# z430/keyword-spotting

Measured on AMD Instinct MI355X. Metric: 1s 16kHz clips/sec end-to-end (wav->label), higher is better.
Workload: dtype f32

## Files before the change

keyword-spotting_amd/csrc/kws_api.hip:

```cpp
#include <atomic>
#include <chrono>
#include <cmath>
#include <cstdio>
#include <cstring>
#include <new>

#include "kws_ctx.h"

namespace kws {

const char* const kKernelNames[KWS_K_COUNT] = {"kws_mfcc_i16_kernel", "kws_dscnn_fwd_kernel", "kws_cnntrad_conv_kernel",
                                               "kws_cnntrad_dense_kernel", "kws_stream_frame_kernel", "kws_mfcc_f64_kernel",
                                               "kws_mfcc_refine_kernel"};


static double hz2mel(double hz) { return 2595.0 * std::log10(1.0 + hz / 700.0); }
static double mel2hz(double mel) { return 700.0 * (std::pow(10.0, mel / 2595.0) - 1.0); }

static void mel_edges(int nfilt, int nfft, int sample_rate, std::vector<int>& edges) {
    const double lowmel = hz2mel(0.0), highmel = hz2mel(sample_rate / 2.0);
    const int num = nfilt + 2;
    const double step = (highmel - lowmel) / (double)(num - 1);
    edges.resize(num);
    for (int i = 0; i < num; ++i) {
// ... 151 lines not shown
    KWS_GUARD_BEGIN
    if (!out) return fail(nullptr, KWS_EINVAL, "kws_create: out is NULL");
    *out = nullptr;
    int ndev = 0;
    hipError_t e = hipGetDeviceCount(&ndev);
    if (e != hipSuccess || ndev <= 0)
        return fail(nullptr, KWS_EHIP, std::string("kws_create: no HIP device (") + hipGetErrorString(e) + "); there is no CPU fallback");
    if (device_id < 0 || device_id >= ndev) return fail(nullptr, KWS_EINVAL, "kws_create: device_id out of range");
    kws_ctx* c = new (std::nothrow) kws_ctx();
    if (!c) return fail(nullptr, KWS_ENOMEM, "kws_create: out of host memory");
    c->device = device_id;
    e = hipSetDevice(device_id);
    if (e == hipSuccess) e = hipStreamCreateWithFlags(&c->own_stream, hipStreamNonBlocking);
    if (e == hipSuccess) e = dscnn_init_device();
    if (e == hipSuccess) e = cnntrad_init_device();
    if (e != hipSuccess) {
        int rc = fail_hip(nullptr, e, "kws_create");
        if (c->own_stream) (void)hipStreamDestroy(c->own_stream);
        delete c;
        return rc;
    }
    c->stream = c->own_stream;
    int rc = kws_set_frontend(c, 16000, 16000, 400, 160, 512, 26, 10, 0.97f, 22);
    if (rc != KWS_OK) {
        g_create_err = c->err;
        kws_destroy(c);
        return rc;
    }
    *out = c;
    return KWS_OK;
// ... 543 lines not shown
    if (rc) return rc;
    if (!d_logits) return fail(c, KWS_EINVAL, std::string(fn) + ": d_logits is NULL");
    if (!c->model_ready) return fail(c, KWS_ESTATE, std::string(fn) + ": no model loaded (kws_load_dscnn)");
    HIP_TRY(c, hipSetDevice(c->device));
    if (c->mw.in_channels > 1) {
        if (d_act || d_stamps || (mode != KWS_PW_SPLIT_BF16 && mode != KWS_PW_PAIR_F16))
            return fail(c, KWS_EUNSUPPORTED, std::string(fn) + ": input_channels > 1 runs on the product kernels only");
        rc = grow_conv_ws(c, (size_t)B * 64 * 141, fn);
        if (rc) return rc;
        HIP_TRY(c, launch_conv1_general(c->stream, d_feat, B, c->mw.in_channels, c->mw.c1_general, c->mw.c1_b, c->d_conv_ws));
        ProfScope ps(c, KWS_K_DSCNN);
        HIP_TRY(c, launch_dscnn(c->stream, c->mw, c->d_conv_ws, B, d_logits, d_label, nullptr, mode, nullptr, nullptr, true));
        return KWS_OK;
    }
    ProfScope ps(c, KWS_K_DSCNN);
    HIP_TRY(c, launch_dscnn(c->stream, c->mw, d_feat, B, d_logits, d_label, d_act, mode, d_stamps));
    return KWS_OK;
}

int kws_forward_f32(kws_ctx* c, const float* d_feat, int B, float* d_logits, int32_t* d_label) {
    return forward_impl(c, d_feat, B, d_logits, d_label, nullptr, c ? c->pw_math : 0, "kws_forward_f32");
}

static int forward_map_impl(kws_ctx* c, const float* d_feat, int B, int T, int F, float* d_logits, int32_t* d_label, float* d_layers,
                            const char* fn) {
    int rc = check_batch(c, d_feat, B, fn);
    if (rc) return rc;
    if (!d_logits) return fail(c, KWS_EINVAL, std::string(fn) + ": d_logits is NULL");
    if (!c->model_ready) return fail(c, KWS_ESTATE, std::string(fn) + ": no model loaded (kws_load_dscnn)");
    if (T == IN_T && F == IN_F && !d_layers) return forward_impl(c, d_feat, B, d_logits, d_label, nullptr, c->pw_math, fn);
    if (T < 6 || F < 6) return fail(c, KWS_EINVAL, std::string(fn) + ": the 10 x 10 first convolution (padding 2) needs T >= 6 and F >= 6");
// ... 1030 lines not shown
```

keyword-spotting_amd/csrc/kws_ctx.h:

```cpp
#pragma once
#include <new>

#include "kws_internal.h"

namespace kws {
struct Ingest;
void ingest_free(kws_ctx* c);
}

using kws::FrontendParams; using kws::FrontendTables; using kws::DscnnWeights; using kws::CnnTradWeights; using kws::NFFT;

struct kws_ctx {
    int device = 0;
    hipStream_t own_stream = nullptr;
    hipStream_t stream = nullptr;
    hipEvent_t order_ev = nullptr;
    std::string err;

    int sample_rate = 16000, nfft = NFFT, ceplifter = 22;
    FrontendParams fp{};
    bool fe_ready = false;
    bool fe_fast_ok = false;
    int fe_math = KWS_FE_F32;
    void* d_fe = nullptr;
    FrontendTables ft{};
    double* d_spec_tw64 = nullptr;
    int spec_nfft = 0;
    float refine_span = KWS_FE_REFINE_SPAN_DEFAULT;
// ... 88 lines not shown
```

keyword-spotting_amd/csrc/kws_dscnn.hip:

```cpp
#include <type_traits>

#include "kws_internal.h"
#include "kws_mfcc_dev.h"
#include "kws_split_mfma.h"

namespace kws {
namespace {


#ifndef KWS_DSCNN_WAVES
#define KWS_DSCNN_WAVES 8
#endif
#ifndef KWS_X_DSCNN_STAMP_TID
#define KWS_X_DSCNN_STAMP_TID 0
#endif
constexpr int NW = KWS_DSCNN_WAVES;
constexpr int NT = NW * 64;
constexpr int TW = 30;

constexpr int P0 = C1_H * C1_W;
constexpr int FEAT_H = 103, FEAT_W = 14;
constexpr int OFF_Z3 = 0, OFF_Z2 = 22976, OFF_Z1 = 0, OFF_Z0 = 9152, OFF_FEAT = 18304;
constexpr int OFF_DWTAB = 38784;
constexpr int OFF_PWB = OFF_DWTAB + 2 * 768;
// ... 23 lines not shown

#ifndef KWS_DSCNN_KSPLIT_LEFTOVER
#define KWS_DSCNN_KSPLIT_LEFTOVER 1
#endif
template <int N>
struct Leftover {
    static constexpr bool HAS = KWS_DSCNN_KSPLIT_LEFTOVER && (N == 1 || N == 2);
    static constexpr int TILE = N == 1 ? 4 : 8;
    static constexpr int P0T = TILE * TW;
    static constexpr int NP = HAS ? Blk<N>::POUT - P0T : 1;
    static constexpr int WAVE0 = N == 1 ? 4 : 0;
    static constexpr int OFF_PART = N == 1 ? OFF_Z2 : OFF_Z0;
};
static_assert(Blk<1>::TILES == 5 && Blk<2>::TILES == 9, "the leftover tiles are the fifth of block 1 and the ninth of block 2");
static_assert(4 * CH * Leftover<1>::NP <= 38784 - OFF_Z2 && OFF_Z0 + 4 * CH * Leftover<2>::NP <= OFF_FEAT, "partial sums fit their dead planes");

template <bool TO_MFMA = false>
__device__ __forceinline__ float stencil3x3(float w0, float w1, float w2, float w3, float w4, float w5, float w6,
                                            float w7, float w8, float b, float up, float mid, float dn, float mask_l,
                                            float mask_r) {
    float c, to_right, to_left;
    asm("v_mul_f32 %1, %3, %13\n\t"
        "v_mul_f32 %2, %5, %13\n\t"
        "v_fma_f32 %0, %4, %13, %12\n\t"
        "v_fmac_f32 %1, %6, %14\n\t"
        "v_fmac_f32 %2, %8, %14\n\t"
        "v_fmac_f32 %0, %7, %14\n\t"
        "v_fmac_f32 %1, %9, %15\n\t"
        "v_fmac_f32 %2, %11, %15\n\t"
        "v_fmac_f32 %0, %10, %15\n\t"
// ... 281 lines not shown
                const int oo = (ct ^ 1) * 32 + row_of(r, half);
                const float u0 = relu(fmaf(w.c1_b[oo], sig0, occ[r])), u1 = relu(fmaf(w.c1_b[oo + 1], sig0, occ[r + 1]));
                *reinterpret_cast<float2*>(z0 + pidx(oo, pos, P0 + 2)) = make_float2(u0, u1);
                if constexpr (PAIR) mx = fmaxf(mx, fmaxf(u0, u1));
            }
        }
    }
}

constexpr int C1W_ROWS = FEAT_H;
constexpr int OFF_C1W8 = OFF_Z1;
constexpr int OFF_C1P2 = OFF_C1W8 + 2 * C1W_ROWS * 3 * 4;
static_assert(OFF_C1P2 + 2 * C1W_ROWS * 3 <= OFF_Z0, "conv1's operand windows live where block 1's output goes later");
static_assert(2 * (C1_W - 1) + 9 < FEAT_W && 2 * (C1_H - 1) + 9 < FEAT_H, "window reach inside the padded map");

__device__ __forceinline__ void conv1_build_windows(float* lds, int tid, float sx) {
    const float* featp = lds + OFF_FEAT;
    uint32_t* w8 = reinterpret_cast<uint32_t*>(lds + OFF_C1W8);
    uint32_t* p2 = reinterpret_cast<uint32_t*>(lds + OFF_C1P2);
    for (int i = tid; i < C1W_ROWS * 3; i += NT) {
        const float* src = featp + (i / 3) * FEAT_W + 2 * (i % 3);
        const float y[8] = {src[0], src[1], src[2], src[3], src[4], src[5], src[6], src[7]};
        uintx4 hi, lo;
        split_pair8(y, sx, hi, lo);
        *reinterpret_cast<uintx4*>(w8 + i * 4) = hi;
        *reinterpret_cast<uintx4*>(w8 + (C1W_ROWS * 3 + i) * 4) = lo;
        uint32_t h, l;
        split_pair2(src[8], src[9], sx, h, l);
        p2[i] = h;
        p2[C1W_ROWS * 3 + i] = l;
    }
}
// ... 71 lines not shown
                const float c0 = (r & 2) ? o4.z : o4.x, c1 = (r & 2) ? o4.w : o4.y;
                const float u0 = relu(fmaf(c0, sig0, occ[r])), u1 = relu(fmaf(c1, sig0, occ[r + 1]));
                *reinterpret_cast<float2*>(z0 + pidx(oo, pos, P0 + 2)) = make_float2(u0, u1);
                mx = fmaxf(mx, fmaxf(u0, u1));
            }
        }
    }
}

struct PosRange {
    int lo, hi;
};

template <bool RANGED, int NP>
__device__ __forceinline__ void conv1_phase_split(const DscnnWeights& w, float* lds, int tid, const uintx4 (&c1f)[7][NP],
                                                  PosRange rg, float sx = 1.f, float sig0 = 1.f) {
    static_assert(P0 > 4 * 32 && P0 <= 5 * 32 && NW >= 6, "conv1 work split: four dual tiles + one tile in two halves");
    const float* featp = lds + OFF_FEAT;
    float* z0 = lds + OFF_Z0;
    const int lane = tid & 63, wv = tid >> 6;
    float mx = 0.f;
    if constexpr (NP == 2) {
        if constexpr (RANGED) {
            const int n_pt = (rg.hi - rg.lo + 31) / 32;
            for (int u = wv; u < 2 * n_pt; u += NW) conv1_unit_pairwin<false>(w, lds, z0, u >> 1, u & 1, lane, c1f, rg.lo, rg.hi, sig0, mx);
        } else if (wv < 4)
            conv1_unit_pairwin<true>(w, lds, z0, wv, wv & 1, lane, c1f, 0, P0, sig0, mx);
        else if (wv < 6)
            conv1_unit_pairwin<false>(w, lds, z0, 4, wv & 1, lane, c1f, 0, P0, sig0, mx);
    } else if constexpr (RANGED) {
        const int n_pt = (rg.hi - rg.lo + 31) / 32;
        for (int u = wv; u < 2 * n_pt; u += NW) conv1_unit_split<false, NP>(w, featp, z0, u >> 1, u & 1, lane, c1f, rg.lo, rg.hi, sx, sig0, mx);
    } else if (wv < 4)
// ... 82 lines not shown
    const float* pwb = lds + OFF_PWB + G::BUF * 64;
    float* zout = lds + G::OFF_OUT;
    float mx = 0.f;
    for (int i = tid; i < CH * L::NP; i += NT) {
        const int co = i / L::NP, j = i - co * L::NP;
        const float s = (part[i] + part[CH * L::NP + i]) + (part[2 * CH * L::NP + i] + part[3 * CH * L::NP + i]);
        const float v = relu(s + pwb[co]);
        zout[pidx(co, L::P0T + j, G::SOUT)] = v;
        mx = fmaxf(mx, v);
    }
    if constexpr (PAIR) publish_wave_max(lds, N == 1 ? 3 : 1, tid >> 6, tid & 63, mx);
}

template <int N, int MODE, bool RANGED = false>
__device__ __forceinline__ void block_phase(const DscnnWeights& w, float* lds, int tid, PwOperands<MODE>& pwo,
                                            float* __restrict__ act4 = nullptr, PosRange rg = PosRange{0, 0}, PairCtx pc = PairCtx{}) {
    using G = Blk<N>;
    constexpr bool PAIR = MODE == 5;
    constexpr int NP = PAIR ? 2 : 3;
    constexpr int NPROD = PAIR ? 3 : 6;
    constexpr bool KSL = Leftover<N>::HAS && (MODE == 4 || MODE == 5) && !RANGED;
    const int p_lo = RANGED ? rg.lo : 0, p_hi = RANGED ? rg.hi : G::POUT;
#ifdef KWS_X_DSCNN_SKIP_LEFTOVER
    const int n_tiles = RANGED ? (p_hi - p_lo + TW - 1) / TW : (N == 2 ? 8 : G::TILES);
#else
    const int n_tiles = RANGED ? (p_hi - p_lo + TW - 1) / TW : (KSL ? Leftover<N>::TILE : G::TILES);
#endif
    constexpr bool MFMA = MODE != 0;
    constexpr bool SPLIT = MODE >= 4;
    constexpr bool NO_STENCIL = MODE == 6;
    const int lane = tid & 63, wv = tid >> 6, half = lane >> 5, col = lane & 31;
    float* zout = lds + G::OFF_OUT;
    const float* dwtab = lds + OFF_DWTAB + G::BUF * 768;
    const float* pwb = lds + OFF_PWB + G::BUF * 64;
    float* poolbuf = lds + OFF_POOLBUF;

    BlockTables next_tables;
    if constexpr (N < 4) {
        fetch_block_tables(w, N + 1, tid, next_tables);
        if (tid < CH) {
            zout[pidx(tid, G::POUT, G::SOUT)] = relu(pwb[tid]);
            zout[pidx(tid, G::POUT + 1, G::SOUT)] = 0.f;
        }
    } else if (!MFMA) {
        poolbuf[wv * CH + lane] = 0.f;
    }

    const float4* bias4 = reinterpret_cast<const float4*>(pwb) + half;
    const float4* dwt4 = reinterpret_cast<const float4*>(dwtab) + half * 24;
    float psum[2][16];
// ... 340 lines not shown
                    "v_add_f32_dpp %12, %12, %12 row_bcast:15 row_mask:0xa bank_mask:0xf\n\t"
                    "v_add_f32_dpp %13, %13, %13 row_bcast:15 row_mask:0xa bank_mask:0xf\n\t"
                    "v_add_f32_dpp %14, %14, %14 row_bcast:15 row_mask:0xa bank_mask:0xf\n\t"
                    "v_add_f32_dpp %15, %15, %15 row_bcast:15 row_mask:0xa bank_mask:0xf"
                    : "+v"(q[0]), "+v"(q[1]), "+v"(q[2]), "+v"(q[3]), "+v"(q[4]), "+v"(q[5]), "+v"(q[6]), "+v"(q[7]), "+v"(q[8]), "+v"(q[9]), "+v"(q[10]), "+v"(q[11]), "+v"(q[12]), "+v"(q[13]), "+v"(q[14]), "+v"(q[15]));
            }
            if (col == 31) {
#pragma unroll
                for (int k = 0; k < 32; ++k) poolbuf[wv * CH + (k >> 4) * 32 + row_of(k & 15, half)] = psum[k >> 4][k & 15] * pc.inv_out;
            }
        }
    }
    (void)bias4;
}


template <int MODE, bool DIAG = true, bool PRECONV = false, bool STREAM = false, bool CLUSTER = false>
__global__ __launch_bounds__(NT) void kws_dscnn_fwd_kernel(DscnnWeights w, const float* __restrict__ feat, int B,
                                                           float* __restrict__ logits, int32_t* __restrict__ label,
                                                           float* __restrict__ act_arg,
                                                           unsigned long long* __restrict__ stamps_arg,
                                                           const int* __restrict__ ring_hops, StreamPush sp) {
    static_assert(!STREAM || (MODE >= 4 && !DIAG && !PRECONV), "the fused push exists for the product paths only");
    constexpr bool PAIR = MODE == 5;
    constexpr int NP = PAIR ? 2 : 3;
    BlockTables t1_pre{};
    static_assert(!CLUSTER || STREAM, "time-tile clusters exist for the streaming push only");
    float* const act = DIAG ? act_arg : nullptr;
    unsigned long long* const stamps = DIAG ? stamps_arg : nullptr;
    extern __shared__ __attribute__((aligned(16))) float lds[];
    constexpr bool MFMA = MODE != 0;
    const int tid = threadIdx.x;
    const int lane = tid & 63, wv = tid >> 6;

    const int cl_n = CLUSTER ? sp.cluster : 1;
    const int clip = CLUSTER ? (int)blockIdx.x / cl_n : (int)blockIdx.x;
    const int cl_tile = CLUSTER ? (int)blockIdx.x - clip * cl_n : 0;
    if (clip >= B) return;
    const int j0 = Blk<4>::H * cl_tile / cl_n, j1 = Blk<4>::H * (cl_tile + 1) / cl_n;
    auto rows = [&](int lo, int hi, int H, int W) { return PosRange{(lo < 0 ? 0 : lo) * W, (hi > H ? H : hi) * W}; };
    const PosRange rg4 = rows(j0, j1, Blk<4>::H, Blk<4>::W), rg3 = rows(j0 - 2, j1, Blk<3>::H, Blk<3>::W),
                   rg2 = rows(j0 - 4, j1, Blk<2>::H, Blk<2>::W), rg1 = rows(j0 - 6, j1, Blk<1>::H, Blk<1>::W),
                   rg0 = rows(j0 - 7, j1 + 1, C1_H, C1_W);
    int n_stamp = 0;
    auto stamp = [&]() {
        if (stamps && tid == KWS_X_DSCNN_STAMP_TID) stamps[(size_t)clip * KWS_DSCNN_STAMPS + n_stamp] = __builtin_amdgcn_s_memtime();
        ++n_stamp;
    };
    if (stamps && tid == KWS_X_DSCNN_STAMP_TID) stamps[(size_t)clip * KWS_DSCNN_STAMPS + KWS_DSCNN_STAMPS - 2] = __builtin_amdgcn_s_memrealtime();
    stamp();

    constexpr bool SPLIT = MODE >= 4;
    PwOperands<MODE> wa;
    int hops_before = 0;
    int kx = 0, ky[5] = {0, 0, 0, 0, 0}, sg[5] = {0, 0, 0, 0, 0};
    if constexpr (PRECONV) {
        static_assert(!PRECONV || MODE >= 4, "the pre-convolved entry exists for the product (split) path only");
        const float* z = feat + (size_t)clip * (CH * P0);
        fetch_block_tables(w, 1, tid, t1_pre);
        float zmax = 0.f;
        for (int i = tid; i < CH * P0; i += NT) {
            const float v = z[i];
            lds[OFF_Z0 + pidx(i / P0, i % P0, P0 + 2)] = v;
            zmax = fmaxf(zmax, v);
        }
        if (tid < CH) {
            lds[OFF_Z0 + pidx(tid, P0, P0 + 2)] = 0.f;
            lds[OFF_Z0 + pidx(tid, P0 + 1, P0 + 2)] = 0.f;
        }
        if constexpr (PAIR)
            publish_wave_max(lds, 1, wv, lane, zmax);
// ... 20 lines not shown
        if (f_start >= 0) row_new = (int)((((f_start / step) - head) % IN_T + IN_T) % IN_T);
    } else {
        head = ring_hops ? (((*ring_hops + 1 - sp.frames_lag) % IN_T) + IN_T) % IN_T : 0;
    }
#pragma unroll
    for (int k = 0; k < FV; ++k) {
        const int i = tid + k * NT;
        fv[k] = (i < IN_T * IN_F && i / IN_F != row_new) ? f[((i / IN_F + head) % IN_T) * IN_F + i % IN_F] : 0.f;
    }
    BlockTables t1;
    fetch_block_tables(w, 1, tid, t1);
    __builtin_amdgcn_sched_barrier(0);
    float a1[SPLIT ? 1 : 50];
    uintx4 c1f[SPLIT ? 7 : 1][NP];
    if constexpr (SPLIT) {
        const uintx4* src = reinterpret_cast<const uintx4*>(PAIR ? w.c1_pair : w.c1_split) + (size_t)(wv & 1) * (7 * NP * 64) + lane;
#pragma unroll
        for (int kb = 0; kb < 7; ++kb)
#pragma unroll
            for (int p = 0; p < NP; ++p) c1f[kb][p] = src[(kb * NP + p) * 64];
    } else if constexpr (MFMA) {
        const int half = lane >> 5, col = lane & 31, ct = wv & 1;
#pragma unroll
        for (int s = 0; s < 50; ++s) a1[s] = w.c1_w[(2 * s + half) * CH + ct * 32 + col];
        load_pointwise(w, 1, lane, wa);
    }
    __builtin_amdgcn_sched_barrier(0);
    if constexpr (PAIR) {
        float m = 0.f;
#pragma unroll
        for (int k = 0; k < FV; ++k) m = fmaxf(m, fabsf(fv[k]));
        publish_wave_max(lds, 0, wv, lane, m);
    }
    if constexpr (STREAM) {
#ifdef KWS_X_STREAM_NO_FRAME
// ... 134 lines not shown
        pc.s_pwb = pow2f(sg[4]);
    }
    block_phase<3, MODE, CLUSTER>(w, lds, tid, wa, nullptr, rg3, pc);
    stamp();
    __syncthreads();
    stamp();
    if (a) {
        const float u = PAIR ? pow2f(-sg[3]) : 1.f;
        for (int i = tid; i < CH * Blk<3>::POUT; i += NT)
            a[i] = lds[OFF_Z3 + pidx(i / Blk<3>::POUT, i % Blk<3>::POUT, Blk<3>::SOUT)] * u;
        a += CH * Blk<3>::POUT;
    }
    if constexpr (PAIR) {
        pc.inv_out = pow2f(-sg[4]);
    }
    block_phase<4, MODE, CLUSTER>(w, lds, tid, wa, a ? a + CH : nullptr, rg4, pc);
    stamp();
    const int C = w.num_classes;
    float4 fcw[CH / 4];
    float fcb = 0.f, ring_b = 0.f;
    if (wv == 0 && lane < C) {
        const float4* wr = reinterpret_cast<const float4*>(w.fc_w + lane * CH);
#pragma unroll
        for (int c = 0; c < CH / 4; ++c) fcw[c] = wr[c];
        fcb = w.fc_b[lane];
    }
    if (tid < CH) ring_b = w.pw_b[3 * CH + tid];
    __syncthreads();
    stamp();

    float* pooled = lds + OFF_POOLED;
    constexpr float RING_N = 55.f * 11.f - 53.f * 9.f;
// ... 44 lines not shown
            const float4* pl = reinterpret_cast<const float4*>(pooled);
#pragma unroll
            for (int c = 0; c < CH / 4; ++c) {
                const float4 a4 = fcw[c], p4 = pl[c];
                acc = fmaf(a4.x, p4.x, acc);
                acc = fmaf(a4.y, p4.y, acc);
                acc = fmaf(a4.z, p4.z, acc);
                acc = fmaf(a4.w, p4.w, acc);
            }
            logits[(size_t)clip * C + lane] = acc;
            if constexpr (STREAM) {
                if (sp.h_logits) __hip_atomic_store(sp.h_logits + (size_t)clip * C + lane, acc, __ATOMIC_RELAXED, __HIP_MEMORY_SCOPE_SYSTEM);
            }
            v = acc;
        }
        float m = v;
        m = fmaxf(m, __builtin_bit_cast(float, __builtin_amdgcn_update_dpp(__builtin_bit_cast(int, m), __builtin_bit_cast(int, m), 0x111, 0xf, 0xf, false)));
        m = fmaxf(m, __builtin_bit_cast(float, __builtin_amdgcn_update_dpp(__builtin_bit_cast(int, m), __builtin_bit_cast(int, m), 0x112, 0xf, 0xf, false)));
        m = fmaxf(m, __builtin_bit_cast(float, __builtin_amdgcn_update_dpp(__builtin_bit_cast(int, m), __builtin_bit_cast(int, m), 0x114, 0xf, 0xf, false)));
        m = fmaxf(m, __builtin_bit_cast(float, __builtin_amdgcn_update_dpp(__builtin_bit_cast(int, m), __builtin_bit_cast(int, m), 0x118, 0xf, 0xf, false)));
        m = fmaxf(m, __builtin_bit_cast(float, __builtin_amdgcn_update_dpp(__builtin_bit_cast(int, m), __builtin_bit_cast(int, m), 0x142, 0xa, 0xf, false)));
        m = fmaxf(m, __builtin_bit_cast(float, __builtin_amdgcn_update_dpp(__builtin_bit_cast(int, m), __builtin_bit_cast(int, m), 0x143, 0xc, 0xf, false)));
        const float vmax = __builtin_bit_cast(float, __builtin_amdgcn_readlane(__builtin_bit_cast(int, m), 63));
        const unsigned long long holders = __ballot(lane < C && v == vmax);
        const int idx = holders ? __ffsll(holders) - 1 : 0;
        if (label && lane == 0) label[clip] = idx;
        if constexpr (STREAM) {
            if (sp.h_label && lane == 0) __hip_atomic_store(sp.h_label + clip, idx, __ATOMIC_RELAXED, __HIP_MEMORY_SCOPE_SYSTEM);
        }
    }
    if constexpr (STREAM) {
        int finishers = (int)gridDim.x;
        if constexpr (CLUSTER) finishers /= cl_n;
        if (sp.h_flag) asm volatile("s_waitcnt vmcnt(0)" ::: "memory");
        if (run_fc && tid == 0 && atomicAdd(&sp.hops[1], 1) == finishers - 1) {
            sp.hops[1] = 0;
            sp.hops[0] = hops_before + 1;
            if (sp.h_flag) __hip_atomic_store(sp.h_flag, hops_before + 1, __ATOMIC_RELAXED, __HIP_MEMORY_SCOPE_SYSTEM);
        }
    }
    stamp();
    if (stamps && tid == KWS_X_DSCNN_STAMP_TID) stamps[(size_t)clip * KWS_DSCNN_STAMPS + KWS_DSCNN_STAMPS - 1] = __builtin_amdgcn_s_memrealtime();
}

}

hipError_t dscnn_init_device() {
    const int lds = LDS_FLOATS * (int)sizeof(float);
    const void* kernels[] = {reinterpret_cast<const void*>(kws_dscnn_fwd_kernel<0>), reinterpret_cast<const void*>(kws_dscnn_fwd_kernel<1>),
                             reinterpret_cast<const void*>(kws_dscnn_fwd_kernel<2>), reinterpret_cast<const void*>(kws_dscnn_fwd_kernel<3>),
                             reinterpret_cast<const void*>(kws_dscnn_fwd_kernel<4>), reinterpret_cast<const void*>(kws_dscnn_fwd_kernel<6>),
                             reinterpret_cast<const void*>(kws_dscnn_fwd_kernel<4, false>),
                             reinterpret_cast<const void*>(kws_dscnn_fwd_kernel<4, false, true>),
                             reinterpret_cast<const void*>(kws_dscnn_fwd_kernel<4, false, false, true>),
                             reinterpret_cast<const void*>(kws_dscnn_fwd_kernel<4, false, false, true, true>),
                             reinterpret_cast<const void*>(kws_dscnn_fwd_kernel<5>), reinterpret_cast<const void*>(kws_dscnn_fwd_kernel<5, false>),
                             reinterpret_cast<const void*>(kws_dscnn_fwd_kernel<5, false, true>),
                             reinterpret_cast<const void*>(kws_dscnn_fwd_kernel<5, false, false, true>),
                             reinterpret_cast<const void*>(kws_dscnn_fwd_kernel<5, false, false, true, true>)};
    for (const void* k : kernels) {
        hipError_t e = hipFuncSetAttribute(k, hipFuncAttributeMaxDynamicSharedMemorySize, lds);
        if (e != hipSuccess) return e;
    }
    return hipSuccess;
}

namespace {
__global__ __launch_bounds__(NT) void kws_conv1_general_kernel(const float* __restrict__ x, int C_in, const float* __restrict__ wt,
                                                               const float* __restrict__ bias, float* __restrict__ out) {
    __shared__ float plane[FEAT_H * FEAT_W];
    const int tid = threadIdx.x, co = tid & 63, g = tid >> 6;
    constexpr int PER = (P0 + NW - 1) / NW;
    float acc[PER];
#pragma unroll
// ... 44 lines not shown
            hipLaunchKernelGGL((kws_dscnn_fwd_kernel<4, false, false, true, true>), dim3(n_streams * sp.cluster), dim3(NT), lds, s, w, d_feat_ring,
                               n_streams, d_logits, d_label, nullptr, nullptr, nullptr, sp);
    } else {
        if (pair)
            hipLaunchKernelGGL((kws_dscnn_fwd_kernel<5, false, false, true>), dim3(n_streams), dim3(NT), lds, s, w, d_feat_ring, n_streams, d_logits,
                               d_label, nullptr, nullptr, nullptr, sp);
        else
            hipLaunchKernelGGL((kws_dscnn_fwd_kernel<4, false, false, true>), dim3(n_streams), dim3(NT), lds, s, w, d_feat_ring, n_streams, d_logits,
                               d_label, nullptr, nullptr, nullptr, sp);
    }
    return hipGetLastError();
}

hipError_t launch_dscnn(hipStream_t s, const DscnnWeights& w, const float* d_feat, int B, float* d_logits,
                        int32_t* d_label, float* d_act, int mode, unsigned long long* d_stamps, const int* d_ring_hops,
                        bool preconv, int frames_lag) {
    const size_t lds = LDS_FLOATS * sizeof(float);
    StreamPush lag{};
    lag.frames_lag = frames_lag;
    const int grid = B;
    if (preconv) {
        if (mode == 5)
            hipLaunchKernelGGL((kws_dscnn_fwd_kernel<5, false, true>), dim3(grid), dim3(NT), lds, s, w, d_feat, B, d_logits, d_label, nullptr, nullptr, nullptr, StreamPush{});
        else
            hipLaunchKernelGGL((kws_dscnn_fwd_kernel<4, false, true>), dim3(grid), dim3(NT), lds, s, w, d_feat, B, d_logits, d_label, nullptr, nullptr, nullptr, StreamPush{});
        return hipGetLastError();
    }
    switch (mode) {
        case 0: hipLaunchKernelGGL(kws_dscnn_fwd_kernel<0>, dim3(grid), dim3(NT), lds, s, w, d_feat, B, d_logits, d_label, d_act, d_stamps, d_ring_hops, lag); break;
        case 2: hipLaunchKernelGGL(kws_dscnn_fwd_kernel<2>, dim3(grid), dim3(NT), lds, s, w, d_feat, B, d_logits, d_label, d_act, d_stamps, d_ring_hops, lag); break;
        case 3: hipLaunchKernelGGL(kws_dscnn_fwd_kernel<3>, dim3(grid), dim3(NT), lds, s, w, d_feat, B, d_logits, d_label, d_act, d_stamps, d_ring_hops, lag); break;
        case 4:
            if (d_act || d_stamps)
                hipLaunchKernelGGL((kws_dscnn_fwd_kernel<4, true>), dim3(grid), dim3(NT), lds, s, w, d_feat, B, d_logits, d_label, d_act, d_stamps, d_ring_hops, lag);
            else
// ... 141 lines not shown
```

keyword-spotting_amd/csrc/kws_internal.h:

```cpp
#pragma once
#include <hip/hip_runtime.h>
#include <stdint.h>

#include <string>
#include <vector>

#include "kws_hip.h"

namespace kws {

constexpr int NFFT = 512;
constexpr int NBINS = NFFT / 2 + 1;
constexpr int MEL_CHUNK = 8;
constexpr int MEL_STRIDE = 10;
#ifndef KWS_MFCC_WAVES
#define KWS_MFCC_WAVES 4
#endif
#ifndef KWS_MFCC_PAIRS_PER_WAVE
#define KWS_MFCC_PAIRS_PER_WAVE 3
#endif
constexpr int MFCC_WAVES = KWS_MFCC_WAVES;
constexpr int MFCC_THREADS = MFCC_WAVES * 64;
constexpr int MFCC_FRAMES_PER_WG = 2 * KWS_MFCC_PAIRS_PER_WAVE * MFCC_WAVES;
constexpr int MAX_NFILT = 64;
// ... 115 lines not shown
    int ring_len;
    int* hops;
    int* refine_ctr;
    int frames_lag;
    int cluster;
    float* cl_part;
    int* cl_count;
    float* h_logits;
    int32_t* h_label;
    int* h_flag;
};
hipError_t launch_dscnn_stream(hipStream_t s, const DscnnWeights& w, const StreamPush& sp, float* d_feat_ring, int n_streams,
                               float* d_logits, int32_t* d_label, bool pair);
hipError_t launch_dscnn(hipStream_t s, const DscnnWeights& w, const float* d_feat, int B, float* d_logits,
                        int32_t* d_label, float* d_act, int mode, unsigned long long* d_stamps = nullptr,
                        const int* d_ring_hops = nullptr, bool preconv = false, int frames_lag = 3);
hipError_t launch_conv1_general(hipStream_t s, const float* d_x, int B, int C_in, const float* d_wt, const float* d_bias, float* d_out);

struct CnnTradWeights {
    const uint32_t* c1_split;
    const float* c1_b;
    const uint32_t* c2_split;
    const float* c2_b;
    const uint32_t* lin_split;
    const float* lin_b;
    const float* dnn_w;
    const float* dnn_b;
    const float* fc_w;
    const float* fc_b;
    int num_classes;
    const uint32_t* c1_h2;
// ... 31 lines not shown
```

Measured before the change: 6.941 million.

## Run DS-CNN forward as persistent workgroups that prefetch the next clip

```diff
diff --git a/keyword-spotting_amd/csrc/kws_api.hip b/keyword-spotting_amd/csrc/kws_api.hip
--- a/keyword-spotting_amd/csrc/kws_api.hip
+++ b/keyword-spotting_amd/csrc/kws_api.hip
@@ -189,6 +189,11 @@
     if (e == hipSuccess) e = hipStreamCreateWithFlags(&c->own_stream, hipStreamNonBlocking);
     if (e == hipSuccess) e = dscnn_init_device();
     if (e == hipSuccess) e = cnntrad_init_device();
+    if (e == hipSuccess) {
+        hipDeviceProp_t prop;
+        e = hipGetDeviceProperties(&prop, device_id);
+        if (e == hipSuccess) c->n_cu = prop.multiProcessorCount;
+    }
     if (e != hipSuccess) {
         int rc = fail_hip(nullptr, e, "kws_create");
         if (c->own_stream) (void)hipStreamDestroy(c->own_stream);
@@ -762,7 +767,7 @@
         return KWS_OK;
     }
     ProfScope ps(c, KWS_K_DSCNN);
-    HIP_TRY(c, launch_dscnn(c->stream, c->mw, d_feat, B, d_logits, d_label, d_act, mode, d_stamps));
+    HIP_TRY(c, launch_dscnn(c->stream, c->mw, d_feat, B, d_logits, d_label, d_act, mode, d_stamps, nullptr, false, 3, c->n_cu));
     return KWS_OK;
 }
 
diff --git a/keyword-spotting_amd/csrc/kws_ctx.h b/keyword-spotting_amd/csrc/kws_ctx.h
--- a/keyword-spotting_amd/csrc/kws_ctx.h
+++ b/keyword-spotting_amd/csrc/kws_ctx.h
@@ -12,6 +12,7 @@
 
 struct kws_ctx {
     int device = 0;
+    int n_cu = 0;
     hipStream_t own_stream = nullptr;
     hipStream_t stream = nullptr;
     hipEvent_t order_ev = nullptr;
diff --git a/keyword-spotting_amd/csrc/kws_dscnn.hip b/keyword-spotting_amd/csrc/kws_dscnn.hip
--- a/keyword-spotting_amd/csrc/kws_dscnn.hip
+++ b/keyword-spotting_amd/csrc/kws_dscnn.hip
@@ -61,6 +61,14 @@
 };
 static_assert(Blk<1>::TILES == 5 && Blk<2>::TILES == 9, "the leftover tiles are the fifth of block 1 and the ninth of block 2");
 static_assert(4 * CH * Leftover<1>::NP <= 38784 - OFF_Z2 && OFF_Z0 + 4 * CH * Leftover<2>::NP <= OFF_FEAT, "partial sums fit their dead planes");
+
+constexpr int OFF_FEAT_P = OFF_Z2;
+constexpr int OFF_POOLBUF_P = OFF_FEAT_P + 1456;
+constexpr int STAGE_WAVES = 4;
+static_assert(OFF_FEAT_P >= OFF_Z3 + Blk<3>::SOUT * CH, "the next clip's features must not overlap block 4's input");
+static_assert(OFF_FEAT_P + FEAT_H * FEAT_W <= OFF_POOLBUF_P && OFF_POOLBUF_P % 4 == 0, "features and pool partials are disjoint");
+static_assert(OFF_POOLBUF_P + NW * CH <= OFF_Z2 + Blk<2>::SOUT * CH && OFF_Z2 + Blk<2>::SOUT * CH <= OFF_DWTAB,
+              "pool partials stay inside the Z2 plane, clear of the table buffers the next clip's block 1 rewrites");
 
 template <bool TO_MFMA = false>
 __device__ __forceinline__ float stencil3x3(float w0, float w1, float w2, float w3, float w4, float w5, float w6,
@@ -372,8 +380,8 @@
 static_assert(OFF_C1P2 + 2 * C1W_ROWS * 3 <= OFF_Z0, "conv1's operand windows live where block 1's output goes later");
 static_assert(2 * (C1_W - 1) + 9 < FEAT_W && 2 * (C1_H - 1) + 9 < FEAT_H, "window reach inside the padded map");
 
-__device__ __forceinline__ void conv1_build_windows(float* lds, int tid, float sx) {
-    const float* featp = lds + OFF_FEAT;
+__device__ __forceinline__ void conv1_build_windows(float* lds, int tid, float sx, int off_feat = OFF_FEAT) {
+    const float* featp = lds + off_feat;
     uint32_t* w8 = reinterpret_cast<uint32_t*>(lds + OFF_C1W8);
     uint32_t* p2 = reinterpret_cast<uint32_t*>(lds + OFF_C1P2);
     for (int i = tid; i < C1W_ROWS * 3; i += NT) {
@@ -475,9 +483,9 @@
 
 template <bool RANGED, int NP>
 __device__ __forceinline__ void conv1_phase_split(const DscnnWeights& w, float* lds, int tid, const uintx4 (&c1f)[7][NP],
-                                                  PosRange rg, float sx = 1.f, float sig0 = 1.f) {
+                                                  PosRange rg, float sx = 1.f, float sig0 = 1.f, int off_feat = OFF_FEAT) {
     static_assert(P0 > 4 * 32 && P0 <= 5 * 32 && NW >= 6, "conv1 work split: four dual tiles + one tile in two halves");
-    const float* featp = lds + OFF_FEAT;
+    const float* featp = lds + off_feat;
     float* z0 = lds + OFF_Z0;
     const int lane = tid & 63, wv = tid >> 6;
     float mx = 0.f;
@@ -590,7 +598,8 @@
 
 template <int N, int MODE, bool RANGED = false>
 __device__ __forceinline__ void block_phase(const DscnnWeights& w, float* lds, int tid, PwOperands<MODE>& pwo,
-                                            float* __restrict__ act4 = nullptr, PosRange rg = PosRange{0, 0}, PairCtx pc = PairCtx{}) {
+                                            float* __restrict__ act4 = nullptr, PosRange rg = PosRange{0, 0}, PairCtx pc = PairCtx{},
+                                            int off_poolbuf = OFF_POOLBUF) {
     using G = Blk<N>;
     constexpr bool PAIR = MODE == 5;
     constexpr int NP = PAIR ? 2 : 3;
@@ -609,7 +618,7 @@
     float* zout = lds + G::OFF_OUT;
     const float* dwtab = lds + OFF_DWTAB + G::BUF * 768;
     const float* pwb = lds + OFF_PWB + G::BUF * 64;
-    float* poolbuf = lds + OFF_POOLBUF;
+    float* poolbuf = lds + off_poolbuf;
 
     BlockTables next_tables;
     if constexpr (N < 4) {
@@ -980,14 +989,110 @@
     (void)bias4;
 }
 
-
-template <int MODE, bool DIAG = true, bool PRECONV = false, bool STREAM = false, bool CLUSTER = false>
-__global__ __launch_bounds__(NT) void kws_dscnn_fwd_kernel(DscnnWeights w, const float* __restrict__ feat, int B,
+template <int NP>
+__device__ __forceinline__ void load_conv1_frags(const DscnnWeights& w, int wv, int lane, uintx4 (&c1f)[7][NP]) {
+    const uintx4* src = reinterpret_cast<const uintx4*>(NP == 2 ? w.c1_pair : w.c1_split) + (size_t)(wv & 1) * (7 * NP * 64) + lane;
+#pragma unroll
+    for (int kb = 0; kb < 7; ++kb)
+#pragma unroll
+        for (int p = 0; p < NP; ++p) c1f[kb][p] = src[(kb * NP + p) * 64];
+}
+
+__device__ __forceinline__ int wave_argmax_first(float v, int lane, int C) {
+    float m = v;
+    m = fmaxf(m, __builtin_bit_cast(float, __builtin_amdgcn_update_dpp(__builtin_bit_cast(int, m), __builtin_bit_cast(int, m), 0x111, 0xf, 0xf, false)));
+    m = fmaxf(m, __builtin_bit_cast(float, __builtin_amdgcn_update_dpp(__builtin_bit_cast(int, m), __builtin_bit_cast(int, m), 0x112, 0xf, 0xf, false)));
+    m = fmaxf(m, __builtin_bit_cast(float, __builtin_amdgcn_update_dpp(__builtin_bit_cast(int, m), __builtin_bit_cast(int, m), 0x114, 0xf, 0xf, false)));
+    m = fmaxf(m, __builtin_bit_cast(float, __builtin_amdgcn_update_dpp(__builtin_bit_cast(int, m), __builtin_bit_cast(int, m), 0x118, 0xf, 0xf, false)));
+    m = fmaxf(m, __builtin_bit_cast(float, __builtin_amdgcn_update_dpp(__builtin_bit_cast(int, m), __builtin_bit_cast(int, m), 0x142, 0xa, 0xf, false)));
+    m = fmaxf(m, __builtin_bit_cast(float, __builtin_amdgcn_update_dpp(__builtin_bit_cast(int, m), __builtin_bit_cast(int, m), 0x143, 0xc, 0xf, false)));
+    const float vmax = __builtin_bit_cast(float, __builtin_amdgcn_readlane(__builtin_bit_cast(int, m), 63));
+    const unsigned long long holders = __ballot(lane < C && v == vmax);
+    return holders ? __ffsll(holders) - 1 : 0;
+}
+
+__device__ __forceinline__ DscnnWeights weights_for_this_clip() {
+#if defined(__HIP_DEVICE_COMPILE__)
+    using KArg = const __attribute__((address_space(4))) DscnnWeights*;
+    KArg p = (KArg)__builtin_amdgcn_kernarg_segment_ptr();
+    asm volatile("" : "+s"(p));
+    return *p;
+#else
+    return DscnnWeights{};
+#endif
+}
+
+template <bool PAIR>
+__device__ __forceinline__ void stage_features_persist(float* lds, const float* __restrict__ feat, int clip, int tid) {
+    constexpr int ST = STAGE_WAVES * 64;
+    constexpr int FV = (IN_T * IN_F + ST - 1) / ST;
+    static_assert(2 * STAGE_WAVES == NW, "each staging wavefront zeroes the maximum slot of one other wavefront");
+    const int lane = tid & 63, wv = tid >> 6;
+    const float* f = feat + (size_t)clip * (IN_T * IN_F);
+    float fv[FV];
+#pragma unroll
+    for (int k = 0; k < FV; ++k) {
+        const int i = tid + k * ST;
+        fv[k] = i < IN_T * IN_F ? f[i] : 0.f;
+    }
+    float* featp = lds + OFF_FEAT_P;
+    for (int i = tid; i < FEAT_H * FEAT_W; i += ST) {
+        const int r = i / FEAT_W - 2, c = i % FEAT_W - 2;
+        if (!((unsigned)r < (unsigned)IN_T && (unsigned)c < (unsigned)IN_F)) featp[i] = 0.f;
+    }
+#pragma unroll
+    for (int k = 0; k < FV; ++k) {
+        const int i = tid + k * ST;
+        if (i < IN_T * IN_F) featp[(i / IN_F + 2) * FEAT_W + (i % IN_F) + 2] = fv[k];
+    }
+    if constexpr (PAIR) {
+        float m = 0.f;
+#pragma unroll
+        for (int k = 0; k < FV; ++k) m = fmaxf(m, fabsf(fv[k]));
+        publish_wave_max(lds, 0, wv, lane, m);
+        if (lane == 63) lds[OFF_WMAX + wv + STAGE_WAVES] = 0.f;
+    }
+}
+
+__device__ __forceinline__ void pool_fc_wave(const DscnnWeights& w, const float* lds, int lane, int clip, float* __restrict__ logits,
+                                             int32_t* __restrict__ label, float* __restrict__ a_pool) {
+    const int C = w.num_classes;
+    float4 fcw[CH / 4];
+    float fcb = 0.f;
+    const float4* wr = reinterpret_cast<const float4*>(w.fc_w + (lane < C ? lane : 0) * CH);
+#pragma unroll
+    for (int c = 0; c < CH / 4; ++c) fcw[c] = wr[c];
+    if (lane < C) fcb = w.fc_b[lane];
+    const float ring_b = w.pw_b[3 * CH + lane];
+    constexpr float RING_N = 55.f * 11.f - 53.f * 9.f;
+    float s = 0.f;
+#pragma unroll
+    for (int k = 0; k < NW; ++k) s += lds[OFF_POOLBUF_P + k * CH + lane];
+    s = fmaf(RING_N, relu(ring_b), s) * (1.0f / (55.f * 11.f));
+    if (a_pool) a_pool[lane] = s;
+    float acc = fcb;
+#pragma unroll
+    for (int c = 0; c < CH / 4; ++c) {
+        const float4 a4 = fcw[c];
+        acc = fmaf(a4.x, __builtin_bit_cast(float, __builtin_amdgcn_readlane(__builtin_bit_cast(int, s), 4 * c + 0)), acc);
+        acc = fmaf(a4.y, __builtin_bit_cast(float, __builtin_amdgcn_readlane(__builtin_bit_cast(int, s), 4 * c + 1)), acc);
+        acc = fmaf(a4.z, __builtin_bit_cast(float, __builtin_amdgcn_readlane(__builtin_bit_cast(int, s), 4 * c + 2)), acc);
+        acc = fmaf(a4.w, __builtin_bit_cast(float, __builtin_amdgcn_readlane(__builtin_bit_cast(int, s), 4 * c + 3)), acc);
+    }
+    if (lane < C) logits[(size_t)clip * C + lane] = acc;
+    const int idx = wave_argmax_first(lane < C ? acc : -INFINITY, lane, C);
+    if (label && lane == 0) label[clip] = idx;
+}
+
+
+template <int MODE, bool DIAG = true, bool PRECONV = false, bool STREAM = false, bool CLUSTER = false, bool PERSIST = false>
+__global__ __launch_bounds__(NT) void kws_dscnn_fwd_kernel(DscnnWeights w_arg, const float* __restrict__ feat, int B,
                                                            float* __restrict__ logits, int32_t* __restrict__ label,
                                                            float* __restrict__ act_arg,
                                                            unsigned long long* __restrict__ stamps_arg,
                                                            const int* __restrict__ ring_hops, StreamPush sp) {
     static_assert(!STREAM || (MODE >= 4 && !DIAG && !PRECONV), "the fused push exists for the product paths only");
+    static_assert(!PERSIST || ((MODE == 4 || MODE == 5) && !PRECONV && !STREAM), "persistent workgroups: batched product paths only");
     constexpr bool PAIR = MODE == 5;
     constexpr int NP = PAIR ? 2 : 3;
     BlockTables t1_pre{};
@@ -996,11 +1101,11 @@
     unsigned long long* const stamps = DIAG ? stamps_arg : nullptr;
     extern __shared__ __attribute__((aligned(16))) float lds[];
     constexpr bool MFMA = MODE != 0;
-    const int tid = threadIdx.x;
-    const int lane = tid & 63, wv = tid >> 6;
+    const int tid_k = threadIdx.x;
+    const int lane_k = tid_k & 63, wv_k = tid_k >> 6;
 
     const int cl_n = CLUSTER ? sp.cluster : 1;
-    const int clip = CLUSTER ? (int)blockIdx.x / cl_n : (int)blockIdx.x;
+    int clip = CLUSTER ? (int)blockIdx.x / cl_n : (int)blockIdx.x;
     const int cl_tile = CLUSTER ? (int)blockIdx.x - clip * cl_n : 0;
     if (clip >= B) return;
     const int j0 = Blk<4>::H * cl_tile / cl_n, j1 = Blk<4>::H * (cl_tile + 1) / cl_n;
@@ -1010,17 +1115,60 @@
                    rg0 = rows(j0 - 7, j1 + 1, C1_H, C1_W);
     int n_stamp = 0;
     auto stamp = [&]() {
-        if (stamps && tid == KWS_X_DSCNN_STAMP_TID) stamps[(size_t)clip * KWS_DSCNN_STAMPS + n_stamp] = __builtin_amdgcn_s_memtime();
+        if (stamps && tid_k == KWS_X_DSCNN_STAMP_TID) stamps[(size_t)clip * KWS_DSCNN_STAMPS + n_stamp] = __builtin_amdgcn_s_memtime();
         ++n_stamp;
     };
+
+    constexpr bool SPLIT = MODE >= 4;
+    BlockTables t1p{};
+    uintx4 c1p[PERSIST ? 7 : 1][NP];
+    int prev_clip = -1;
+    float* a_prev = nullptr;
+    if constexpr (PERSIST) {
+        fetch_block_tables(w_arg, 1, tid_k, t1p);
+        if (wv_k < STAGE_WAVES) stage_features_persist<PAIR>(lds, feat, clip, tid_k);
+        load_conv1_frags(w_arg, wv_k, lane_k, c1p);
+        __syncthreads();
+    }
+    for (;;) {
+    const DscnnWeights w = PERSIST ? weights_for_this_clip() : w_arg;
+    int tid = tid_k;
+    if constexpr (PERSIST) {
+        int wv_l = __builtin_amdgcn_readfirstlane(wv_k), lane_l = lane_k;
+        asm volatile("" : "+s"(wv_l), "+v"(lane_l));
+        tid = (wv_l << 6) | (lane_l & 63);
+    }
+    const int lane = tid & 63, wv = tid >> 6;
+    if constexpr (PERSIST) n_stamp = 0;
     if (stamps && tid == KWS_X_DSCNN_STAMP_TID) stamps[(size_t)clip * KWS_DSCNN_STAMPS + KWS_DSCNN_STAMPS - 2] = __builtin_amdgcn_s_memrealtime();
     stamp();
 
-    constexpr bool SPLIT = MODE >= 4;
     PwOperands<MODE> wa;
     int hops_before = 0;
     int kx = 0, ky[5] = {0, 0, 0, 0, 0}, sg[5] = {0, 0, 0, 0, 0};
-    if constexpr (PRECONV) {
+    if constexpr (PERSIST) {
+        if constexpr (PAIR) {
+            const float mxf = read_stage_max(lds, 0, 1);
+            kx = pow2_exp_for(mxf);
+            const float bz0 = (w.c1_abs * mxf + w.c1_bmax) * 1.001f;
+            cap_units(kx, sg[0], w.k_c1, bz0);
+            const float by1 = (w.dw_abs[0] * bz0 + w.dw_bmax[0]) * 1.001f;
+            ky[1] = pow2_exp_for(by1);
+            cap_units(ky[1], sg[1], w.k_pw[0], (w.pw_abs[0] * by1 + w.pw_bmax[0]) * 1.001f);
+            store_block_tables(lds, 1, tid, t1p, pow2f(ky[1]), pow2f(sg[1]), pow2f(ky[1] - sg[0]));
+            conv1_build_windows(lds, tid, pow2f(kx), OFF_FEAT_P);
+            __syncthreads();
+        } else {
+            store_block_tables(lds, 1, tid, t1p);
+        }
+        stamp();
+        conv1_phase_split<false, NP>(w, lds, tid, c1p, rg0, pow2f(kx), pow2f(sg[0]), OFF_FEAT_P);
+        if (wv == NW - 1 && prev_clip >= 0) {
+            pool_fc_wave(w, lds, lane, prev_clip, logits, label, a_prev);
+            if (stamps && lane == 0) stamps[(size_t)prev_clip * KWS_DSCNN_STAMPS + 13] = __builtin_amdgcn_s_memtime();
+        }
+        load_afrag(w, 1, wv >= 4 ? wv - 4 : 0, lane, wa.ring[0]);
+    } else if constexpr (PRECONV) {
         static_assert(!PRECONV || MODE >= 4, "the pre-convolved entry exists for the product (split) path only");
         const float* z = feat + (size_t)clip * (CH * P0);
         fetch_block_tables(w, 1, tid, t1_pre);
@@ -1071,11 +1219,7 @@
     float a1[SPLIT ? 1 : 50];
     uintx4 c1f[SPLIT ? 7 : 1][NP];
     if constexpr (SPLIT) {
-        const uintx4* src = reinterpret_cast<const uintx4*>(PAIR ? w.c1_pair : w.c1_split) + (size_t)(wv & 1) * (7 * NP * 64) + lane;
-#pragma unroll
-        for (int kb = 0; kb < 7; ++kb)
-#pragma unroll
-            for (int p = 0; p < NP; ++p) c1f[kb][p] = src[(kb * NP + p) * 64];
+        load_conv1_frags(w, wv, lane, c1f);
     } else if constexpr (MFMA) {
         const int half = lane >> 5, col = lane & 31, ct = wv & 1;
 #pragma unroll
@@ -1240,8 +1384,24 @@
     if constexpr (PAIR) {
         pc.inv_out = pow2f(-sg[4]);
     }
-    block_phase<4, MODE, CLUSTER>(w, lds, tid, wa, a ? a + CH : nullptr, rg4, pc);
+    block_phase<4, MODE, CLUSTER>(w, lds, tid, wa, a ? a + CH : nullptr, rg4, pc,
+                                  PERSIST ? OFF_POOLBUF_P : OFF_POOLBUF);
     stamp();
+    if constexpr (PERSIST) {
+        const int next = clip + (int)gridDim.x;
+        __builtin_amdgcn_sched_barrier(0);
+        if (wv < STAGE_WAVES && next < B) stage_features_persist<PAIR>(lds, feat, next, tid);
+        stamp();
+        load_conv1_frags(w, wv, lane, c1p);
+        __syncthreads();
+        stamp();
+        if (stamps && tid == KWS_X_DSCNN_STAMP_TID) stamps[(size_t)clip * KWS_DSCNN_STAMPS + KWS_DSCNN_STAMPS - 1] = __builtin_amdgcn_s_memrealtime();
+        prev_clip = clip;
+        a_prev = a;
+        clip = next;
+        if (clip >= B) break;
+        continue;
+    }
     const int C = w.num_classes;
     float4 fcw[CH / 4];
     float fcb = 0.f, ring_b = 0.f;
@@ -1316,16 +1476,7 @@
             }
             v = acc;
         }
-        float m = v;
-        m = fmaxf(m, __builtin_bit_cast(float, __builtin_amdgcn_update_dpp(__builtin_bit_cast(int, m), __builtin_bit_cast(int, m), 0x111, 0xf, 0xf, false)));
-        m = fmaxf(m, __builtin_bit_cast(float, __builtin_amdgcn_update_dpp(__builtin_bit_cast(int, m), __builtin_bit_cast(int, m), 0x112, 0xf, 0xf, false)));
-        m = fmaxf(m, __builtin_bit_cast(float, __builtin_amdgcn_update_dpp(__builtin_bit_cast(int, m), __builtin_bit_cast(int, m), 0x114, 0xf, 0xf, false)));
-        m = fmaxf(m, __builtin_bit_cast(float, __builtin_amdgcn_update_dpp(__builtin_bit_cast(int, m), __builtin_bit_cast(int, m), 0x118, 0xf, 0xf, false)));
-        m = fmaxf(m, __builtin_bit_cast(float, __builtin_amdgcn_update_dpp(__builtin_bit_cast(int, m), __builtin_bit_cast(int, m), 0x142, 0xa, 0xf, false)));
-        m = fmaxf(m, __builtin_bit_cast(float, __builtin_amdgcn_update_dpp(__builtin_bit_cast(int, m), __builtin_bit_cast(int, m), 0x143, 0xc, 0xf, false)));
-        const float vmax = __builtin_bit_cast(float, __builtin_amdgcn_readlane(__builtin_bit_cast(int, m), 63));
-        const unsigned long long holders = __ballot(lane < C && v == vmax);
-        const int idx = holders ? __ffsll(holders) - 1 : 0;
+        const int idx = wave_argmax_first(v, lane, C);
         if (label && lane == 0) label[clip] = idx;
         if constexpr (STREAM) {
             if (sp.h_label && lane == 0) __hip_atomic_store(sp.h_label + clip, idx, __ATOMIC_RELAXED, __HIP_MEMORY_SCOPE_SYSTEM);
@@ -1343,6 +1494,14 @@
     }
     stamp();
     if (stamps && tid == KWS_X_DSCNN_STAMP_TID) stamps[(size_t)clip * KWS_DSCNN_STAMPS + KWS_DSCNN_STAMPS - 1] = __builtin_amdgcn_s_memrealtime();
+    break;
+    }
+    if constexpr (PERSIST) {
+        if (wv_k == NW - 1) {
+            pool_fc_wave(w_arg, lds, lane_k, prev_clip, logits, label, a_prev);
+            if (stamps && lane_k == 0) stamps[(size_t)prev_clip * KWS_DSCNN_STAMPS + 13] = __builtin_amdgcn_s_memtime();
+        }
+    }
 }
 
 }
@@ -1359,7 +1518,11 @@
                              reinterpret_cast<const void*>(kws_dscnn_fwd_kernel<5>), reinterpret_cast<const void*>(kws_dscnn_fwd_kernel<5, false>),
                              reinterpret_cast<const void*>(kws_dscnn_fwd_kernel<5, false, true>),
                              reinterpret_cast<const void*>(kws_dscnn_fwd_kernel<5, false, false, true>),
-                             reinterpret_cast<const void*>(kws_dscnn_fwd_kernel<5, false, false, true, true>)};
+                             reinterpret_cast<const void*>(kws_dscnn_fwd_kernel<5, false, false, true, true>),
+                             reinterpret_cast<const void*>(kws_dscnn_fwd_kernel<4, true, false, false, false, true>),
+                             reinterpret_cast<const void*>(kws_dscnn_fwd_kernel<4, false, false, false, false, true>),
+                             reinterpret_cast<const void*>(kws_dscnn_fwd_kernel<5, true, false, false, false, true>),
+                             reinterpret_cast<const void*>(kws_dscnn_fwd_kernel<5, false, false, false, false, true>)};
     for (const void* k : kernels) {
         hipError_t e = hipFuncSetAttribute(k, hipFuncAttributeMaxDynamicSharedMemorySize, lds);
         if (e != hipSuccess) return e;
@@ -1434,11 +1597,23 @@
 
 hipError_t launch_dscnn(hipStream_t s, const DscnnWeights& w, const float* d_feat, int B, float* d_logits,
                         int32_t* d_label, float* d_act, int mode, unsigned long long* d_stamps, const int* d_ring_hops,
-                        bool preconv, int frames_lag) {
+                        bool preconv, int frames_lag, int n_cu) {
     const size_t lds = LDS_FLOATS * sizeof(float);
     StreamPush lag{};
     lag.frames_lag = frames_lag;
     const int grid = B;
+    if (n_cu > 0 && B > n_cu && !preconv && !d_ring_hops && (mode == 4 || mode == 5)) {
+        const bool diag = d_act || d_stamps;
+        if (mode == 5 && diag)
+            hipLaunchKernelGGL((kws_dscnn_fwd_kernel<5, true, false, false, false, true>), dim3(n_cu), dim3(NT), lds, s, w, d_feat, B, d_logits, d_label, d_act, d_stamps, nullptr, lag);
+        else if (mode == 5)
+            hipLaunchKernelGGL((kws_dscnn_fwd_kernel<5, false, false, false, false, true>), dim3(n_cu), dim3(NT), lds, s, w, d_feat, B, d_logits, d_label, nullptr, nullptr, nullptr, lag);
+        else if (diag)
+            hipLaunchKernelGGL((kws_dscnn_fwd_kernel<4, true, false, false, false, true>), dim3(n_cu), dim3(NT), lds, s, w, d_feat, B, d_logits, d_label, d_act, d_stamps, nullptr, lag);
+        else
+            hipLaunchKernelGGL((kws_dscnn_fwd_kernel<4, false, false, false, false, true>), dim3(n_cu), dim3(NT), lds, s, w, d_feat, B, d_logits, d_label, nullptr, nullptr, nullptr, lag);
+        return hipGetLastError();
+    }
     if (preconv) {
         if (mode == 5)
             hipLaunchKernelGGL((kws_dscnn_fwd_kernel<5, false, true>), dim3(grid), dim3(NT), lds, s, w, d_feat, B, d_logits, d_label, nullptr, nullptr, nullptr, StreamPush{});
diff --git a/keyword-spotting_amd/csrc/kws_internal.h b/keyword-spotting_amd/csrc/kws_internal.h
--- a/keyword-spotting_amd/csrc/kws_internal.h
+++ b/keyword-spotting_amd/csrc/kws_internal.h
@@ -153,7 +153,7 @@
                                float* d_logits, int32_t* d_label, bool pair);
 hipError_t launch_dscnn(hipStream_t s, const DscnnWeights& w, const float* d_feat, int B, float* d_logits,
                         int32_t* d_label, float* d_act, int mode, unsigned long long* d_stamps = nullptr,
-                        const int* d_ring_hops = nullptr, bool preconv = false, int frames_lag = 3);
+                        const int* d_ring_hops = nullptr, bool preconv = false, int frames_lag = 3, int n_cu = 0);
 hipError_t launch_conv1_general(hipStream_t s, const float* d_x, int B, int C_in, const float* d_wt, const float* d_bias, float* d_out);
 
 struct CnnTradWeights {
```

New measurement: 7.053 million (median of 6 runs). 1.02x the previous value.
